# xiaoyeli/superlu_dist

Hardware: AMD Instinct MI355X
Metric: LU factorization GFLOP/s (pdgstrf3d) + solve time (higher is better)
Workload: dtype f64

## Files before the change

superlu_dist_amd/csrc/sluamd_kernels.hip:

```cpp
#include <hip/hip_runtime.h>
#include <cassert>
#include <cstdio>
#include "sluamd_internal.h"

namespace sluamd {

typedef double d4 __attribute__((ext_vector_type(4)));

__device__ __forceinline__ int find_node(const int *__restrict__ prefix, int nn, int id)
{
    int lo = 0, hi = nn;
    while (hi - lo > 1) {
        int mid = (lo + hi) >> 1;
        if (prefix[mid] <= id) lo = mid; else hi = mid;
    }
    return lo;
}

#ifndef SLUAMD_FIND_WAVE
#define SLUAMD_FIND_WAVE 1
#endif
__device__ __forceinline__ int find_node_wave(const int *__restrict__ prefix, int nn, int id)
{
#if SLUAMD_FIND_WAVE
// ... 475 lines not shown
                        }
#pragma unroll
                        for (int r = 0; r < 4; ++r) {
                            const int col = cg + lk + 4 * r;
                            if (col < ns) { A[jb + li + (size_t) col * lda] = o0[r]; A[jb + 16 + li + (size_t) col * lda] = o1[r]; }
                        }
                    }
                }
        }
        __threadfence_block();
        __syncthreads();
    }
}

__global__ __launch_bounds__(128) void k_diag_inv(DevTables T, const int *__restrict__ nodes,
                                                  const int *__restrict__ prefix, int nn)
{
    __builtin_amdgcn_s_setprio(3);
    __shared__ double Bs[4][DB * (DB + 1)];
    const int g = threadIdx.x >> 5, c = threadIdx.x & 31;
    const int task = blockIdx.x * 4 + g;
    bool valid = task < prefix[nn];
    int k = 0, typ = 0, b = 0, ns = 0, lda = 1, nblk = 1;
    const double *A = nullptr;
    int ni = 0;
    if (valid) {
        ni = find_node(prefix, nn, task);
        k = nodes[ni];
        if (!(T.sn_flags[k] & SNF_HAS_DIAG)) valid = false;
    }
    if (valid) {
        ns = T.xsup[k + 1] - T.xsup[k];
        nblk = (ns + DB - 1) / DB;
        const int rem = task - prefix[ni];
        typ = rem / nblk; b = rem - typ * nblk;
        lda = T.sn_dlda[k];
        A = T.val + T.sn_dptr[k];
    }
    const int o = b * DB;
    if (valid) {
        for (int i = 0; i < DB; ++i) {
            double v = (i == c) ? 1.0 : 0.0;
            if (o + i < ns && o + c < ns && i <= c) {
                if (typ == 0) v = A[o + i + (size_t) (o + c) * lda];
                else if (i < c) v = A[o + c + (size_t) (o + i) * lda];
            }
            Bs[g][i * (DB + 1) + c] = v;
        }
    }
    __syncthreads();
    if (valid) {
        double xi[DB];
#pragma unroll
        for (int i = 0; i < DB; ++i) xi[i] = 0.0;
#pragma unroll
        for (int i = DB - 1; i >= 0; --i) {
            double a = (i == c) ? 1.0 : 0.0;
#pragma unroll
            for (int jj = i + 1; jj < DB; ++jj) a -= Bs[g][i * (DB + 1) + jj] * xi[jj];
            xi[i] = (i <= c) ? a / Bs[g][i * (DB + 1) + i] : 0.0;
        }
        double *dst = T.dinv + T.sn_dinv[k] + (size_t) (typ * nblk + b) * DB * DB + c * DB;
#pragma unroll
        for (int i = 0; i < DB; ++i) dst[i] = xi[i];
    }
}

template <int NG>
__global__ __launch_bounds__(NG * 32) void k_diag_inv_all(DevTables T, const int *__restrict__ nodes)
{
    __shared__ double Bs[NG][DB * (DB + 1)];
    const int k = nodes[blockIdx.x];
    if (!(T.sn_flags[k] & SNF_OWN_DIAG)) return;
    const int ns = T.xsup[k + 1] - T.xsup[k], nblk = (ns + DB - 1) / DB, lda = T.sn_dlda[k];
    const double *A = T.val + T.sn_dptr[k];
    const int g = threadIdx.x >> 5, c = threadIdx.x & 31;
    for (int t0 = 0; t0 < 2 * nblk; t0 += NG) {
        const int task = t0 + g;
        const bool valid = task < 2 * nblk;
        const int typ = task / nblk, b = task - typ * nblk, o = b * DB;
        if (valid)
            for (int i = 0; i < DB; ++i) {
                double v = (i == c) ? 1.0 : 0.0;
                if (o + i < ns && o + c < ns && i <= c) {
                    if (typ == 0) v = A[o + i + (size_t) (o + c) * lda];
                    else if (i < c) v = A[o + c + (size_t) (o + i) * lda];
                }
                Bs[g][i * (DB + 1) + c] = v;
            }
        __syncthreads();
        if (valid) {
            double xi[DB];
#pragma unroll
            for (int i = 0; i < DB; ++i) xi[i] = 0.0;
#pragma unroll
            for (int i = DB - 1; i >= 0; --i) {
                double a = (i == c) ? 1.0 : 0.0;
#pragma unroll
                for (int jj = i + 1; jj < DB; ++jj) a -= Bs[g][i * (DB + 1) + jj] * xi[jj];
                xi[i] = (i <= c) ? a / Bs[g][i * (DB + 1) + i] : 0.0;
            }
            double *dst = T.dinv + T.sn_dinv[k] + (size_t) (typ * nblk + b) * DB * DB + c * DB;
#pragma unroll
            for (int i = 0; i < DB; ++i) dst[i] = xi[i];
        }
        __syncthreads();
    }
}

constexpr int TB_SZ = DB * 48;
static inline size_t trsm_lds_bytes(int rs, int nsp) { return sizeof(double) * ((size_t) rs * nsp + 2 * TB_SZ); }

template <int MODE, int RSv>
__device__ __forceinline__ void panel_trsm_body(const DevTables &T, int k, int strip, double *sm)
{
    constexpr int NT = RSv * 4;
    constexpr int PQ = DB * DB / NT;
    constexpr int ES = NT / 32;
    const int klst = T.xsup[k + 1], ns = klst - T.xsup[k];
    const int nsp = (ns + DB - 1) & ~(DB - 1);
    const int lda = T.sn_nsupr[k];
    const int ldd = T.sn_dlda[k];
    const int nblk = nsp / DB;
    double *A = T.val + T.sn_lval[k];
    const double *Dg = T.val + T.sn_dptr[k];
    double *Uv = T.val + T.sn_uval[k];
    constexpr bool TU = (MODE == 0 || MODE == 3);
    const double *dinv = T.dinv + T.sn_dinv[k] + (TU ? 0 : (size_t) nblk * DB * DB);
    double *Xs = sm;
    double *Tb = sm + (size_t) RSv * nsp;
    const int tid = threadIdx.x, wave = tid >> 6, lane = tid & 63;
    int *s_cp = reinterpret_cast<int *>(Tb), *s_ld = s_cp + RSv;
    auto locate = [&]() {
        if (tid < RSv) {
            const int cr = strip * RSv + tid;
            int cp = 0, ld = nsp;
            if (cr < T.sn_ncolu[k]) { ld = T.ucol_ld[T.sn_ucol[k] + cr]; cp = T.ucol_cp[T.sn_ucol[k] + cr]; }
            s_cp[tid] = cp; s_ld[tid] = ld;
        }
        __syncthreads();
    };

    if (MODE >= 2) {
        const int row0 = strip * RSv;
        for (int idx = tid; idx < RSv * nsp; idx += NT) {
            const int r = idx % RSv, c = idx / RSv;
            Xs[((r >> 4) * nsp + c) * 16 + (r & 15)] = (row0 + r == c && c < ns) ? 1.0 : 0.0;
        }
    } else if (MODE == 0) {
        const int row0 = T.sn_ldiag[k] + strip * RSv;
#pragma unroll 8
        for (int idx = tid; idx < RSv * nsp; idx += NT) {
            const int r = idx % RSv, c = idx / RSv;
            double v = 0.0;
            if (c < ns && row0 + r < lda) v = A[row0 + r + (size_t) c * lda];
            Xs[((r >> 4) * nsp + c) * 16 + (r & 15)] = v;
        }
    } else {
        locate();
        for (int idx = tid; idx < RSv * nsp; idx += NT) {
            const int c = idx % nsp, r = idx / nsp;
            double v = 0.0;
            const int ld = s_ld[r];
            if (c >= ld && c < ns) v = Uv[s_cp[r] + (c - ld)];
            Xs[((r >> 4) * nsp + c) * 16 + (r & 15)] = v;
        }
        __syncthreads();
    }

    const int e0 = tid & 31, e1 = tid >> 5;
    auto fetch = [&](double *pv, int jb, int t) {
        if (t * DB < jb) {
            const int kc = t * DB;
#pragma unroll
            for (int q = 0; q < PQ; ++q) {
                const int kg = kc + (TU ? e0 : e1 + ES * q), cg = jb + (TU ? e1 + ES * q : e0);
                pv[q] = (kg < ns && cg < ns) ? (TU ? Dg[kg + (size_t) cg * ldd] : Dg[cg + (size_t) kg * ldd]) : 0.0;
            }
        } else {
            const double *dblk = dinv + (size_t) (jb / DB) * DB * DB;
#pragma unroll
            for (int q = 0; q < PQ; ++q) pv[q] = dblk[(e1 + ES * q) * DB + e0];
        }
    };
    auto stash = [&](const double *pv, int jb, int t, int buf) {
        double *tb = Tb + buf * TB_SZ;
#pragma unroll
        for (int q = 0; q < PQ; ++q) {
            if (t * DB < jb && !TU) tb[(e1 + ES * q) * 48 + e0] = pv[q];
            else tb[(e1 + ES * q) * 34 + e0] = pv[q];
        }
    };
    auto advance = [&](int &jb, int &t) { if (++t > jb / DB) { jb += DB; t = 0; } };

    d4 acc0 = (d4){0.0, 0.0, 0.0, 0.0}, acc1 = (d4){0.0, 0.0, 0.0, 0.0};
    const double *xa = Xs + ((size_t) wave * nsp + (lane >> 4)) * 16 + (lane & 15);
    auto compute = [&](int jb, int t, int buf) {
        const bool cfast = !TU && (t < jb / DB);
        const int sk = cfast ? 48 : 1, sc = cfast ? 1 : 34;
        const double *tb0 = Tb + buf * TB_SZ + (lane >> 4) * sk + (lane & 15) * sc;
        const double *tb1 = tb0 + 16 * sc;
        const int ks = 4 * sk;
        if (t < jb / DB) {
            const double *a = xa + (size_t) (t * DB) * 16;
#pragma unroll
            for (int k4 = 0; k4 < DB; k4 += 4) {
                const double av = a[k4 * 16];
                acc0 = __builtin_amdgcn_mfma_f64_16x16x4f64(av, tb0[(k4 >> 2) * ks], acc0, 0, 0, 0);
                acc1 = __builtin_amdgcn_mfma_f64_16x16x4f64(av, tb1[(k4 >> 2) * ks], acc1, 0, 0, 0);
            }
        } else {
            double *x0 = Xs + ((size_t) wave * nsp + jb + (lane & 15)) * 16 + (lane >> 4);
            double *x1 = x0 + 16 * 16;
#pragma unroll
            for (int r = 0; r < 4; ++r) { x0[4 * r] -= acc0[r]; x1[4 * r] -= acc1[r]; }
            acc0 = (d4){0.0, 0.0, 0.0, 0.0}; acc1 = (d4){0.0, 0.0, 0.0, 0.0};
            const double *a = xa + (size_t) jb * 16;
#pragma unroll
            for (int k4 = 0; k4 < DB; k4 += 4) {
                const double av = a[k4 * 16];
                acc0 = __builtin_amdgcn_mfma_f64_16x16x4f64(av, tb0[(k4 >> 2) * ks], acc0, 0, 0, 0);
                acc1 = __builtin_amdgcn_mfma_f64_16x16x4f64(av, tb1[(k4 >> 2) * ks], acc1, 0, 0, 0);
            }
#pragma unroll
            for (int r = 0; r < 4; ++r) { x0[4 * r] = acc0[r]; x1[4 * r] = acc1[r]; }
            acc0 = (d4){0.0, 0.0, 0.0, 0.0}; acc1 = (d4){0.0, 0.0, 0.0, 0.0};
        }
    };

    double pA[PQ], pB[PQ];
    int cj = 0, ct = 0;
    int nj = 0, nt = 0;
    int fj = 0, ft = 0;
    fetch(pA, 0, 0);
    stash(pA, 0, 0, 0);
    advance(nj, nt);
    fj = nj; ft = nt; advance(fj, ft);
    if (nj < nsp) fetch(pA, nj, nt);
    if (fj < nsp) fetch(pB, fj, ft);
    __syncthreads();
    int buf = 0;
    while (cj < nsp) {
        compute(cj, ct, buf);
        if (nj < nsp) stash(pA, nj, nt, buf ^ 1);
        cj = nj; ct = nt; nj = fj; nt = ft; advance(fj, ft);
        if (fj < nsp) fetch(pA, fj, ft);
        __syncthreads();
        buf ^= 1;
        if (cj >= nsp) break;
        compute(cj, ct, buf);
        if (nj < nsp) stash(pB, nj, nt, buf ^ 1);
        cj = nj; ct = nt; nj = fj; nt = ft; advance(fj, ft);
        if (fj < nsp) fetch(pB, fj, ft);
        __syncthreads();
        buf ^= 1;
    }

    if (MODE >= 2) {
        double *out = T.inv + T.sn_inv[k] + (MODE == 3 ? (size_t) ns * ns : 0);
        const int row0 = strip * RSv;
        for (int idx = tid; idx < RSv * ns; idx += NT) {
            const int r = idx % RSv, c = idx / RSv;
            if (row0 + r < ns) out[MODE == 3 ? (row0 + r) + (size_t) c * ns : c + (size_t) (row0 + r) * ns] = Xs[((r >> 4) * nsp + c) * 16 + (r & 15)];
        }
    } else if (MODE == 0) {
        const int row0 = T.sn_ldiag[k] + strip * RSv;
#pragma unroll 8
        for (int idx = tid; idx < RSv * ns; idx += NT) {
            const int r = idx % RSv, c = idx / RSv;
            if (row0 + r < lda) A[row0 + r + (size_t) c * lda] = Xs[((r >> 4) * nsp + c) * 16 + (r & 15)];
        }
    } else {
        locate();
        for (int idx = tid; idx < RSv * nsp; idx += NT) {
            const int c = idx % nsp, r = idx / nsp;
            const int ld = s_ld[r];
            if (c >= ld && c < ns) Uv[s_cp[r] + (c - ld)] = Xs[((r >> 4) * nsp + c) * 16 + (r & 15)];
        }
    }
}

template <int RSv>
__global__ __launch_bounds__(RSv * 4) void k_panel_trsm(DevTables T, const int *__restrict__ nodes,
                                                        const int *__restrict__ lprefix, const int *__restrict__ uprefix,
                                                        int nn, int nl, const int2 *__restrict__ units)
{
    extern __shared__ double sm[];
    if (units) {
        const int2 u = units[blockIdx.x];
        if ((int) blockIdx.x < nl) panel_trsm_body<0, RSv>(T, u.x, u.y, sm);
        else panel_trsm_body<1, RSv>(T, u.x, u.y, sm);
        return;
    }
    if ((int) blockIdx.x < nl) {
        const int ni = find_node_wave(lprefix, nn, blockIdx.x);
        panel_trsm_body<0, RSv>(T, nodes[ni], blockIdx.x - lprefix[ni], sm);
    } else {
        const int id = blockIdx.x - nl;
        const int ni = find_node_wave(uprefix, nn, id);
        panel_trsm_body<1, RSv>(T, nodes[ni], id - uprefix[ni], sm);
    }
}

constexpr int PGK = 64;
constexpr int PG_LDS = PGK * 48;
template <int MODE, int NQ>
__device__ __forceinline__ void panel_gemm_wg(const DevTables &T, int k, int unit64, double *Ts)
{
    const int tid = threadIdx.x, wave = tid >> 6, lane = tid & 63;
    const int unit = unit64 * 4 + wave;
    const int klst = T.xsup[k + 1], ns = klst - T.xsup[k];
    const int nblk = (ns + DB - 1) / DB;
    const int li = lane & 15, lk = lane >> 4;
    double a[NQ];
    const int lda = T.sn_nsupr[k];
    double *A = T.val + T.sn_lval[k];
    double *Uv = T.val + T.sn_uval[k];
    int row = 0, cp = 0, ld = ns;
    bool valid;
    if (MODE == 0) {
        row = T.sn_ldiag[k] + unit * 16 + li;
        valid = row < lda;
    } else {
        const int cr = unit * 16 + li;
        valid = cr < T.sn_ncolu[k];
        if (valid) { ld = T.ucol_ld[T.sn_ucol[k] + cr]; cp = T.ucol_cp[T.sn_ucol[k] + cr]; }
    }
#pragma unroll
    for (int q = 0; q < NQ; ++q) {
        const int c = 4 * q + lk;
        double v = 0.0;
        if (q < nblk * 8) {
            if (MODE == 0) { if (valid && c < ns) v = A[row + (size_t) c * lda]; }
            else { if (valid && c >= ld && c < ns) v = Uv[cp + (c - ld)]; }
        }
        a[q] = v;
    }
    const double *Ti = T.inv + T.sn_inv[k] + (MODE == 0 ? (size_t) ns * ns : 0);
    for (int jb = 0; jb < nblk; ++jb) {
        d4 acc0 = (d4){0.0, 0.0, 0.0, 0.0}, acc1 = (d4){0.0, 0.0, 0.0, 0.0};
#pragma unroll
        for (int kc = 0; kc < NQ / 16; ++kc) {
            if (kc * 2 <= jb) {
                __syncthreads();
                const int k0 = kc * PGK;
                if (MODE == 0) {
#pragma unroll
                    for (int e = 0; e < PGK * DB / 256; ++e) {
                        const int idx = tid + 256 * e, kk = idx & (PGK - 1), np = idx >> 6;
                        const int kg = k0 + kk, n = jb * DB + np;
                        Ts[np * (PGK + 2) + kk] = (kg < ns && n < ns) ? Ti[kg + (size_t) n * ns] : 0.0;
                    }
                } else {
#pragma unroll
                    for (int e = 0; e < PGK * DB / 256; ++e) {
                        const int idx = tid + 256 * e, np = idx & 31, kk = idx >> 5;
                        const int kg = k0 + kk, n = jb * DB + np;
                        Ts[kk * 48 + np] = (kg < ns && n < ns) ? Ti[n + (size_t) kg * ns] : 0.0;
                    }
                }
                __syncthreads();
#pragma unroll
                for (int qq = 0; qq < 16; ++qq) {
                    const int kl = 4 * qq + lk;
                    const double t0 = MODE == 0 ? Ts[li * (PGK + 2) + kl] : Ts[kl * 48 + li];
                    const double t1 = MODE == 0 ? Ts[(16 + li) * (PGK + 2) + kl] : Ts[kl * 48 + 16 + li];
                    acc0 = __builtin_amdgcn_mfma_f64_16x16x4f64(t0, a[16 * kc + qq], acc0, 0, 0, 0);
                    acc1 = __builtin_amdgcn_mfma_f64_16x16x4f64(t1, a[16 * kc + qq], acc1, 0, 0, 0);
                }
            }
        }
#pragma unroll
        for (int r = 0; r < 4; ++r) {
            const int c0 = jb * DB + lk + 4 * r, c1 = c0 + 16;
            if (MODE == 0) {
                if (valid && c0 < ns) A[row + (size_t) c0 * lda] = acc0[r];
                if (valid && c1 < ns) A[row + (size_t) c1 * lda] = acc1[r];
            } else {
                if (valid && c0 >= ld && c0 < ns) Uv[cp + (c0 - ld)] = acc0[r];
                if (valid && c1 >= ld && c1 < ns) Uv[cp + (c1 - ld)] = acc1[r];
            }
        }
    }
}

template <int NQ>
__global__ __launch_bounds__(256) void k_panel_gemm(DevTables T, const int *__restrict__ nodes, const int *__restrict__ lprefix,
                                                    const int *__restrict__ uprefix, int nn, int nl, const int2 *__restrict__ units)
{
    __builtin_amdgcn_s_setprio(3);
    __shared__ double Ts[PG_LDS];
    if (units) {
        const int2 u = units[blockIdx.x];
        if ((int) blockIdx.x < nl) panel_gemm_wg<0, NQ>(T, u.x, u.y, Ts);
        else panel_gemm_wg<1, NQ>(T, u.x, u.y, Ts);
        return;
    }
    if ((int) blockIdx.x < nl) {
        const int ni = find_node_wave(lprefix, nn, blockIdx.x);
        panel_gemm_wg<0, NQ>(T, nodes[ni], blockIdx.x - lprefix[ni], Ts);
    } else {
        const int id = blockIdx.x - nl;
        const int ni = find_node_wave(uprefix, nn, id);
        panel_gemm_wg<1, NQ>(T, nodes[ni], id - uprefix[ni], Ts);
    }
}

constexpr int FIS = 16;
__global__ __launch_bounds__(FIS * 4) void k_full_inv(DevTables T, const int *__restrict__ nodes, const int *__restrict__ prefix, int nn)
{
    __builtin_amdgcn_s_setprio(3);
    extern __shared__ double sm[];
    const int ni = find_node_wave(prefix, nn, blockIdx.x);
    const int k = nodes[ni];
    const int ns = T.xsup[k + 1] - T.xsup[k];
    const int per = (ns + FIS - 1) / FIS;
    const int u = blockIdx.x - prefix[ni];
    if (u < per) panel_trsm_body<2, FIS>(T, k, u, sm);
    else panel_trsm_body<3, FIS>(T, k, u - per, sm);
}

__global__ __launch_bounds__(256) void k_full_inv64(DevTables T, const int *__restrict__ nodes, const int *__restrict__ prefix, int nn)
{
    const int w = blockIdx.x * 4 + (threadIdx.x >> 6);
    const int ni = w >> 1, typ = w & 1;
    if (ni >= nn || prefix[ni + 1] == prefix[ni]) return;
    const int k = nodes[ni];
    const int ns = T.xsup[k + 1] - T.xsup[k], nblk = (ns + DB - 1) / DB, lda = T.sn_dlda[k];
    const double *A = T.val + T.sn_dptr[k];
    const double *D0 = T.dinv + T.sn_dinv[k] + (size_t) (typ * nblk) * DB * DB, *D1 = D0 + DB * DB;
    double *out = T.inv + T.sn_inv[k] + (typ == 0 ? (size_t) ns * ns : 0);
    const int lane = threadIdx.x & 63, li = lane & 15, lk = lane >> 4;
    auto put = [&](int r, int c, double v) { if (r < ns && c < ns) out[typ == 0 ? r + (size_t) c * ns : c + (size_t) r * ns] = v; };
    for (int e = lane; e < DB * DB; e += 64) {
        const int i = e & 31, c = e >> 5;
        put(i, c, D0[c * DB + i]);
        if (nblk == 2) { put(DB + i, DB + c, D1[c * DB + i]); put(DB + i, c, 0.0); }
    }
    if (nblk < 2) return;
    d4 t[2][2];
#pragma unroll
    for (int it = 0; it < 2; ++it)
#pragma unroll
        for (int jt = 0; jt < 2; ++jt) {
            d4 acc = (d4){0.0, 0.0, 0.0, 0.0};
#pragma unroll
            for (int q = 0; q < 8; ++q) {
                const int i = 16 * it + li, kk = 4 * q + lk;
                double a = 0.0;
                if (DB + kk < ns) a = (typ == 0) ? A[i + (size_t) (DB + kk) * lda] : A[(DB + kk) + (size_t) i * lda];
                const double b = D1[(16 * jt + li) * DB + kk];
                acc = __builtin_amdgcn_mfma_f64_16x16x4f64(a, b, acc, 0, 0, 0);
            }
            t[it][jt] = acc;
        }
#pragma unroll
    for (int it = 0; it < 2; ++it)
#pragma unroll
        for (int jt = 0; jt < 2; ++jt) {
            d4 acc = (d4){0.0, 0.0, 0.0, 0.0};
#pragma unroll
            for (int kt = 0; kt < 2; ++kt)
#pragma unroll
                for (int q = 0; q < 4; ++q) {
                    const double a = D0[(16 * kt + 4 * q + lk) * DB + 16 * it + li];
                    acc = __builtin_amdgcn_mfma_f64_16x16x4f64(a, t[kt][jt][q], acc, 0, 0, 0);
                }
#pragma unroll
            for (int r = 0; r < 4; ++r) put(16 * it + lk + 4 * r, DB + 16 * jt + li, -acc[r]);
        }
}

__global__ __launch_bounds__(256) void k_rfs_residual(int n, const int *__restrict__ rp, const int *__restrict__ ci,
                                                      const double *__restrict__ av, const double *__restrict__ x,
                                                      const double *__restrict__ b, const int *__restrict__ pc,
                                                      double *__restrict__ r_perm, unsigned long long *__restrict__ s_out,
                                                      double safe1, double safe2)
{
    __shared__ double red[4];
    const int i = blockIdx.x * 256 + threadIdx.x;
    double q = 0.0;
    if (i < n) {
        double ax = 0.0, t = 0.0;
        for (int e = rp[i]; e < rp[i + 1]; ++e) {
            const double a = av[e], xv = x[ci[e]];
            ax += a * xv;
            t += fabs(a) * fabs(xv);
        }
        const double r = b[i] - ax;
        t += fabs(b[i]);
        r_perm[pc[i]] = r;
        if (t > safe2) q = fabs(r) / t;
        else if (t != 0.0) q = (safe1 + fabs(r)) / t;
    }
#pragma unroll
    for (int o = 32; o > 0; o >>= 1) q = fmax(q, __shfl_xor(q, o));
    if ((threadIdx.x & 63) == 0) red[threadIdx.x >> 6] = q;
    __syncthreads();
    if (threadIdx.x == 0) {
        q = fmax(fmax(red[0], red[1]), fmax(red[2], red[3]));
        atomicMax(s_out, (unsigned long long) __double_as_longlong(q));
    }
}

__global__ __launch_bounds__(256) void k_rfs_update(int n, const int *__restrict__ pc, const double *__restrict__ dx_perm,
                                                    double *__restrict__ x)
{
    const int i = blockIdx.x * 256 + threadIdx.x;
    if (i < n) x[i] += dx_perm[pc[i]];
}


typedef const volatile double __attribute__((address_space(3))) *lds_vdouble_t;
template <int RA, int CA, int LDL, int LDU, bool USW>
__device__ __forceinline__ void schur_chunk(const double *Lb, const double *Ub, int rm0, int cn0, int lane, d4 (&acc)[CA][RA], int pa)
{
#pragma unroll
    for (int k4 = 0; k4 < KC; k4 += 4) {
        const int kr = k4 + (lane >> 4);
        double a[CA], b[RA];
#pragma unroll
        for (int c = 0; c < CA; ++c) a[c] = USW ? ((lds_vdouble_t) Ub)[(pa ^ k4) + 256 * c] : Ub[kr * LDU + cn0 + 16 * c + (lane & 15)];
#pragma unroll
        for (int r = 0; r < RA; ++r) b[r] = USW ? ((lds_vdouble_t) Lb)[kr * LDL + rm0 + 16 * r + (lane & 15)] : Lb[kr * LDL + rm0 + 16 * r + (lane & 15)];
#pragma unroll
        for (int c = 0; c < CA; ++c)
#pragma unroll
            for (int r = 0; r < RA; ++r) acc[c][r] = __builtin_amdgcn_mfma_f64_16x16x4f64(a[c], b[r], acc[c][r], 0, 0, 0);
    }
}

#ifndef SLUAMD_EXP_EPI
#define SLUAMD_EXP_EPI 2
#endif
#ifndef SLUAMD_EXP_NOLOAD
#define SLUAMD_EXP_NOLOAD 0
#endif
#ifndef SLUAMD_EXP_VALU
#define SLUAMD_EXP_VALU 0
#endif
#ifndef SLUAMD_SCHUR_FETCH2
#define SLUAMD_SCHUR_FETCH2 1
#endif
#ifndef SLUAMD_SCHUR_FETCH3
#define SLUAMD_SCHUR_FETCH3 1
#endif
typedef int i32x4 __attribute__((ext_vector_type(4)));
__device__ i32x4 llvm_amdgcn_raw_buffer_load_i32x4(i32x4 rsrc, int voffset, int soffset, int aux) __asm("llvm.amdgcn.raw.buffer.load.v4i32");
__device__ __forceinline__ i32x4 buffer_rsrc(const void *p)
{
    const uint64_t v = (uint64_t) p;
    i32x4 r;
    r.x = __builtin_amdgcn_readfirstlane((int) (uint32_t) v);
    r.y = __builtin_amdgcn_readfirstlane((int) ((uint32_t) (v >> 32) & 0xFFFFu));
    r.z = (int) 0xFFFFFFFFu;
    r.w = 0x00020000;
    return r;
}
__device__ __forceinline__ void lds_dma_16(i32x4 rsrc, uint32_t lds_byte, int voffset, int soffset)
{
    unsigned keep;
    asm volatile("s_mov_b32 %0, m0\n\ts_mov_b32 m0, %4\n\ts_nop 0\n\tbuffer_load_dwordx4 %1, %2, %3 offen lds\n\ts_mov_b32 m0, %0"
                 : "=&s"(keep) : "v"(voffset), "s"(rsrc), "s"(soffset), "s"(lds_byte) : "memory");
}
#ifdef SLUAMD_EXP_NODMAWAIT
__device__ __forceinline__ void lds_dma_wait() { asm volatile("" ::: "memory"); }
#else
__device__ __forceinline__ void lds_dma_wait() { asm volatile("s_waitcnt vmcnt(0)" ::: "memory"); }
#endif
__device__ __forceinline__ uint32_t lds_byte_addr(const void *p) { return (uint32_t) (uintptr_t) (__attribute__((address_space(3))) const void *) p; }
#ifndef SLUAMD_SCHUR_TOUCH
#define SLUAMD_SCHUR_TOUCH 0
#endif
#ifndef SLUAMD_SCHUR_TIGHT
#define SLUAMD_SCHUR_TIGHT 1
#endif
#ifndef SLUAMD_SCHUR_DMA
#define SLUAMD_SCHUR_DMA 1
#endif
#ifndef SLUAMD_SCHUR_CLEAN
#define SLUAMD_SCHUR_CLEAN 1
#endif
typedef double d2 __attribute__((ext_vector_type(2)));
typedef const d2 __attribute__((address_space(1), aligned(8))) *gd2_t;
typedef const char __attribute__((address_space(1))) *gbytes_t;
typedef const double __attribute__((address_space(1))) *gdouble_t;
__device__ __forceinline__ gbytes_t uniform_ptr(const double *p)
{
    const uint64_t v = (uint64_t) p;
    const uint32_t lo = __builtin_amdgcn_readfirstlane((uint32_t) v), hi = __builtin_amdgcn_readfirstlane((uint32_t) (v >> 32));
    return (gbytes_t) (((uint64_t) hi << 32) | lo);
}
#ifndef SCHUR64_WGS
#define SCHUR64_WGS 5
#endif
template <int TMv, int TNv, int NW, bool Z = false, int MM = 0, bool SK = false>
__global__ __launch_bounds__(NW * 64, (NW == 8 ? 4 : (TMv == 128 ? 2 : (Z ? 6 : SCHUR64_WGS)))) void k_schur(DevTables T, const int *__restrict__ nodes,
                                                                    const int *__restrict__ prefix, int nn, int id_base,
                                                                    int ntiles, int *__restrict__ info,
                                                                    const int4 *__restrict__ ulist, int prio,
                                                                    const int *__restrict__ tmaps, const int *__restrict__ xoff)
{
    constexpr int LDL = TMv + 16;
    constexpr int LDU = TNv + 17;
    constexpr int NT = NW * 64;
    constexpr int WR = (NW == 8) ? 4 : 2, WC = 2;
    constexpr int NBR = TMv / (16 * WR), NBC = TNv / (16 * WC);
    constexpr int LQ = TMv * KC / NT, UQ = TNv * KC / NT;
    constexpr int LKS = NT / TMv;
    constexpr int UJS = NT / 16;
    constexpr int ZS = Z ? 2 : 1;
    static_assert(!Z || (LKS % 2 == 0 && KC % 2 == 0), "complex L loader: the parity of a thread's k must be constant");
    constexpr int NBUF = (TMv == 64 && SCHUR64_WGS > 4) ? 1 : 2;
    __shared__ double Ls[NBUF][KC * LDL];
    constexpr bool USW = SLUAMD_SCHUR_FETCH3 && !Z;
    __shared__ __attribute__((aligned(16))) double Us[NBUF][USW ? KC * TNv : KC * LDU];
    auto uidx = [](int k, int c) { return USW ? c * 16 + ((((k >> 1) ^ ((c >> 1) & 7)) << 1) | (k & 1)) : k * LDU + c; };
    __shared__ int s_ind[256 + 8];
    __shared__ int s_rowmap[TMv];
    __shared__ int s_colmap[TNv];
    __shared__ int s_cptr[TNv];
    __shared__ int s_lead[TNv];
    __shared__ int s_cptr2[TNv];
    __shared__ int s_lead2[TNv];
    __shared__ int s_jj[TNv];
    __shared__ int s_dinfo[1];
    __shared__ int s_sink[(SLUAMD_SCHUR_TOUCH == 2 && TMv == 128) ? NW * 64 : 1];
    constexpr int HDR = 64;
    __shared__ int s_hdr[HDR];
    constexpr int REC = HDR + TMv + 3 * TNv;

    const int tid = threadIdx.x;
    int bid;
    if (xoff) {
        const int x = blockIdx.x & 7;
        const int b0 = xoff[x], b1 = xoff[x + 1];
        bid = b0 + (int) (blockIdx.x >> 3);
        if (bid >= b1) return;
        bid += id_base;
    } else {
        const int chunk = (ntiles + 7) >> 3;
        bid = (blockIdx.x & 7) * chunk + (blockIdx.x >> 3);
        if ((blockIdx.x >> 3) >= chunk || bid >= ntiles) return;
        bid += id_base;
    }
    int k, nr, nc, ns, lda, stc, Rw, kbeg_own;
    bool has_dst;
    const double *Lp, *Uv;
    double *dst;
    if (prio) __builtin_amdgcn_s_setprio(2);
    if (MM == 2) {
        const int *rec = tmaps + (size_t) (bid - id_base) * REC;
        for (int t = tid; t < REC; t += NT) {
            const int v = rec[t];
            if (t < HDR) s_hdr[t] = v;
            else if (t < HDR + TMv) s_rowmap[t - HDR] = v;
            else if (t < HDR + TMv + TNv) s_colmap[t - HDR - TMv] = v;
            else if (t < HDR + TMv + 2 * TNv) s_cptr[t - HDR - TMv - TNv] = v;
            else s_lead[t - HDR - TMv - 2 * TNv] = v;
        }
        __syncthreads();
        k = s_hdr[0];
        nr = __builtin_amdgcn_readfirstlane(s_hdr[1]); nc = __builtin_amdgcn_readfirstlane(s_hdr[2]);
        ns = s_hdr[3]; lda = s_hdr[4]; kbeg_own = s_hdr[5];
        Lp = T.val + (((int64_t) s_hdr[7] << 32) | (uint32_t) s_hdr[6]);
        Uv = T.val + (((int64_t) s_hdr[9] << 32) | (uint32_t) s_hdr[8]);
        const int64_t dbase = ((int64_t) s_hdr[11] << 32) | (uint32_t) s_hdr[10];
        has_dst = dbase >= 0;
        dst = T.val + (has_dst ? dbase : 0);
        stc = s_hdr[12]; Rw = s_hdr[13];
        if (!has_dst && tid == 0) atomicAdd(&info[2], 1);
    } else {
        int ib, jb, dblk = -2;
        int4 R, C;
        const int *lsub;
        if (ulist) {
            const int4 u = ulist[bid];
            k = u.x; dblk = u.w;
            R = T.rtile[u.y]; C = T.ctile[u.z];
            const int2 ri = T.rt_info[u.y];
            const int4 ci = T.ct_info[u.z];
            ib = ri.x; jb = ci.x; stc = ci.z;
            lsub = (dblk == -3) ? T.lrow + T.sn_lrow[k] + R.w : T.lidx + ri.y;
        } else {
            const int ni = find_node(prefix, nn, bid);
            k = nodes[ni];
            const int local = bid - prefix[ni];
            const int nct = T.sn_nct[k];
            const int rt = local / nct, ct = local - rt * nct;
            R = T.rtile[T.sn_rt_off[k] + rt];
            C = T.ctile[T.sn_ct_off[k] + ct];
            const int lb = T.sn_lb_off[k] + R.x, ub = T.sn_ub_off[k] + C.x;
            ib = T.lb_gid[lb]; jb = T.ub_gid[ub];
            lsub = T.lidx + T.sn_lidx[k] + T.lb_lptr[lb] + R.y;
// ... 1928 lines not shown
```

Before: 47840.

## Double-buffer inverse tiles in panel GEMM with vectorized prefetch

Restructures the panel GEMM's LDS staging of the diagonal-block inverse into a double-buffered pipeline with 32-wide k-chunks. The next tile is prefetched into registers while MFMAs run on the current buffer, which removes one barrier per chunk. When the inverse is 16-byte aligned and ns is even, loads become double2. The aim is to hide global-load latency behind compute, at the cost of more iterations and registers; a smaller chunk also means finer triangular skipping.

```diff
diff --git a/superlu_dist_amd/csrc/sluamd_kernels.hip b/superlu_dist_amd/csrc/sluamd_kernels.hip
--- a/superlu_dist_amd/csrc/sluamd_kernels.hip
+++ b/superlu_dist_amd/csrc/sluamd_kernels.hip
@@ -801,8 +801,10 @@
     }
 }
 
-constexpr int PGK = 64;
-constexpr int PG_LDS = PGK * 48;
+constexpr int PGK = 32;
+constexpr int PG_LD0 = PGK + 2, PG_LD1 = 48;
+constexpr int PG_BUF = PGK * PG_LD1;
+constexpr int PG_LDS = 2 * PG_BUF;
 template <int MODE, int NQ>
 __device__ __forceinline__ void panel_gemm_wg(const DevTables &T, int k, int unit64, double *Ts)
 {
@@ -836,37 +838,57 @@
         a[q] = v;
     }
     const double *Ti = T.inv + T.sn_inv[k] + (MODE == 0 ? (size_t) ns * ns : 0);
+    constexpr int LD = MODE == 0 ? PG_LD0 : PG_LD1;
+    const bool wide = ((ns & 1) == 0) && ((reinterpret_cast<size_t>(Ti) & 15) == 0);
+    const int f2 = (tid & 15) * 2, s0 = tid >> 4;
+    auto fetch = [&](double (&r)[4], int jb, int kb) {
+        const int F0 = (MODE == 0 ? kb : jb) * DB + f2, S0 = (MODE == 0 ? jb : kb) * DB + s0;
+        if (wide && jb * DB + DB <= ns) {
+#pragma unroll
+            for (int e = 0; e < 2; ++e) {
+                const double2 v = *reinterpret_cast<const double2 *>(Ti + F0 + (size_t) (S0 + 16 * e) * ns);
+                r[2 * e] = v.x; r[2 * e + 1] = v.y;
+            }
+        } else {
+#pragma unroll
+            for (int e = 0; e < 2; ++e) {
+                const int S = S0 + 16 * e;
+                const double *p = Ti + F0 + (size_t) S * ns;
+                r[2 * e] = (F0 < ns && S < ns) ? p[0] : 0.0;
+                r[2 * e + 1] = (F0 + 1 < ns && S < ns) ? p[1] : 0.0;
+            }
+        }
+    };
+    auto stash = [&](const double (&r)[4], int buf) {
+#pragma unroll
+        for (int e = 0; e < 2; ++e)
+            *reinterpret_cast<double2 *>(Ts + buf * PG_BUF + (s0 + 16 * e) * LD + f2) = make_double2(r[2 * e], r[2 * e + 1]);
+    };
+    double r[4];
+    fetch(r, 0, 0);
+    stash(r, 0);
+    __syncthreads();
+    int buf = 0;
     for (int jb = 0; jb < nblk; ++jb) {
         d4 acc0 = (d4){0.0, 0.0, 0.0, 0.0}, acc1 = (d4){0.0, 0.0, 0.0, 0.0};
 #pragma unroll
-        for (int kc = 0; kc < NQ / 16; ++kc) {
-            if (kc * 2 <= jb) {
+        for (int kb = 0; kb < NQ / 8; ++kb) {
+            if (kb <= jb) {
+                const int njb = kb == jb ? jb + 1 : jb, nkb = kb == jb ? 0 : kb + 1;
+                const bool more = njb < nblk;
+                if (more) fetch(r, njb, nkb);
+                const double *Tc = Ts + buf * PG_BUF;
+#pragma unroll
+                for (int qq = 0; qq < 8; ++qq) {
+                    const int kl = 4 * qq + lk;
+                    const double t0 = MODE == 0 ? Tc[li * LD + kl] : Tc[kl * LD + li];
+                    const double t1 = MODE == 0 ? Tc[(16 + li) * LD + kl] : Tc[kl * LD + 16 + li];
+                    acc0 = __builtin_amdgcn_mfma_f64_16x16x4f64(t0, a[8 * kb + qq], acc0, 0, 0, 0);
+                    acc1 = __builtin_amdgcn_mfma_f64_16x16x4f64(t1, a[8 * kb + qq], acc1, 0, 0, 0);
+                }
+                if (more) stash(r, buf ^ 1);
                 __syncthreads();
-                const int k0 = kc * PGK;
-                if (MODE == 0) {
-#pragma unroll
-                    for (int e = 0; e < PGK * DB / 256; ++e) {
-                        const int idx = tid + 256 * e, kk = idx & (PGK - 1), np = idx >> 6;
-                        const int kg = k0 + kk, n = jb * DB + np;
-                        Ts[np * (PGK + 2) + kk] = (kg < ns && n < ns) ? Ti[kg + (size_t) n * ns] : 0.0;
-                    }
-                } else {
-#pragma unroll
-                    for (int e = 0; e < PGK * DB / 256; ++e) {
-                        const int idx = tid + 256 * e, np = idx & 31, kk = idx >> 5;
-                        const int kg = k0 + kk, n = jb * DB + np;
-                        Ts[kk * 48 + np] = (kg < ns && n < ns) ? Ti[n + (size_t) kg * ns] : 0.0;
-                    }
-                }
-                __syncthreads();
-#pragma unroll
-                for (int qq = 0; qq < 16; ++qq) {
-                    const int kl = 4 * qq + lk;
-                    const double t0 = MODE == 0 ? Ts[li * (PGK + 2) + kl] : Ts[kl * 48 + li];
-                    const double t1 = MODE == 0 ? Ts[(16 + li) * (PGK + 2) + kl] : Ts[kl * 48 + 16 + li];
-                    acc0 = __builtin_amdgcn_mfma_f64_16x16x4f64(t0, a[16 * kc + qq], acc0, 0, 0, 0);
-                    acc1 = __builtin_amdgcn_mfma_f64_16x16x4f64(t1, a[16 * kc + qq], acc1, 0, 0, 0);
-                }
+                buf ^= 1;
             }
         }
 #pragma unroll
@@ -888,7 +910,7 @@
                                                     const int *__restrict__ uprefix, int nn, int nl, const int2 *__restrict__ units)
 {
     __builtin_amdgcn_s_setprio(3);
-    __shared__ double Ts[PG_LDS];
+    __shared__ __attribute__((aligned(16))) double Ts[PG_LDS];
     if (units) {
         const int2 u = units[blockIdx.x];
         if ((int) blockIdx.x < nl) panel_gemm_wg<0, NQ>(T, u.x, u.y, Ts);
```

Result: faster. 49200 (median of 6 runs) (+2.8%).
